# liaoherui/StrainScan

Measured on AMD Instinct MI355X. Metric: M reads/sec vs 1433-strain E. coli DB, higher is better.
Workload: dtype u64

## Files before the change

### strainscan_amd/csrc/ss_reorder.hip

```cpp
#include "ss_common.h"

#include <mutex>
#include "ss_scan_dev.h"

#include <hipcub/hipcub.hpp>

#include <algorithm>
#include <chrono>
#include <vector>

namespace {

constexpr int CH = 64;
constexpr int RB = 256 * CH;
constexpr int HALO = 512;
constexpr int MAX_ORDER_BITS = 22;
constexpr uint32_t NO_NL = 0xFFFFFFFFu;
constexpr int TCAP = 2 * CH;

__device__ __forceinline__ uint32_t nl_mask16(const uint4 v)
{
    const uint32_t w[4] = {v.x, v.y, v.z, v.w};
    uint32_t z[4];
#pragma unroll
// ... 205 lines not shown
        first = false;
        if (!more) break;
        __syncthreads();
    }
}


__device__ __forceinline__ void pad_piece(uint32_t (&w)[4], uint32_t rlen, uint32_t c)
{
    const int keep = (int)min(16u, rlen > c ? rlen - c : 0u);
    if (keep < 16) {
#pragma unroll
        for (int d = 0; d < 4; d++) {
            const int k = keep - 4 * d;
            if (k <= 0) w[d] = 0x0A0A0A0Au;
            else if (k < 4) { const uint32_t m = (1u << (8 * k)) - 1u; w[d] = (w[d] & m) | (0x0A0A0A0Au & ~m); }
        }
    }
}

__device__ __forceinline__ int piece_record(const TileLds &L, uint32_t cnt, uint32_t p)
{
    int lo = 0, hi = (int)cnt - 1;
    while (lo < hi) {
        const int mid = (lo + hi) >> 1;
        if (L.pend[mid] <= p) lo = mid + 1; else hi = mid;
    }
    return lo;
}

__device__ __forceinline__ void store_piece(char *__restrict__ dst, uint64_t out, uint4 v, uint32_t rlen, uint32_t rslot, uint32_t c)
{
    uint32_t w[4] = {v.x, v.y, v.z, v.w};
    pad_piece(w, rlen, c);
    char *o8 = static_cast<char *>(__builtin_assume_aligned(dst + out, 8));
    if (c + 16 <= rslot) __builtin_memcpy(o8, w, 16);
    else __builtin_memcpy(o8, w, 8);
}

__device__ __forceinline__ void copy_round(const char *__restrict__ b, uint64_t n, char *__restrict__ dst, TileLds &L, uint32_t cnt)
{
    const int t = threadIdx.x, lane = t & 63, wave = t >> 6;
    const uint32_t pieces = (uint32_t)t < cnt ? (slot_of(L.len[t]) + 15u) >> 4 : 0u;
    uint32_t pend = wave_incl_sum(pieces, lane);
    if (lane == 63) L.wcnt[wave] = pend;
    __syncthreads();
    uint32_t total = 0;
    for (int w = 0; w < 4; w++) { const uint32_t c = L.wcnt[w]; if (w < wave) pend += c; total += c; }
    if ((uint32_t)t < cnt) L.pend[t] = pend;
    __syncthreads();
    for (uint32_t p = (uint32_t)t; p < total; p += 256) {
        const int lo = piece_record(L, cnt, p);
        const uint32_t rlen = L.len[lo], rslot = slot_of(rlen), c = (p - (L.pend[lo] - ((rslot + 15u) >> 4))) * 16u;
        const uint4 x = rlen > c ? load16_nl(b, L.src[lo] + c, n) : make_uint4(0x0A0A0A0Au, 0x0A0A0A0Au, 0x0A0A0A0Au, 0x0A0A0A0Au);
        store_piece(dst, L.dst[lo] + c, x, rlen, rslot, c);
    }
}

constexpr int PRE = 6;
__global__ __launch_bounds__(256, 8) __attribute__((amdgpu_num_sgpr(80))) void place_kernel(
    const char *__restrict__ b, uint64_t n, unsigned long long *__restrict__ cursor, const uint32_t *__restrict__ tab_cnt,
    const unsigned long long *__restrict__ tab, char *__restrict__ dst)
{
    __shared__ TileLds L;
    const int t = threadIdx.x, lane = t & 63, wave = t >> 6;
    static_assert(TCAP <= 256, "one table entry per thread");
    const unsigned long long e = t < TCAP ? tab[(uint64_t)blockIdx.x * TCAP + t] : 0ull;
    const uint32_t known = tab_cnt[blockIdx.x];
    if (known == T_OVERFLOW || known == 0) return;
    uint64_t d0 = 0;
    uint32_t pieces = 0;
    if ((uint32_t)t < known) {
        const uint32_t len = (uint32_t)(e >> START_BITS) & (LEN_LIMIT - 1u);
        L.src[t] = (uint64_t)blockIdx.x * RB + (uint32_t)(e & (uint32_t)(RB - 1));
        L.len[t] = len;
        d0 = atomicAdd(&cursor[(uint32_t)(e >> (START_BITS + LEN_BITS))], (unsigned long long)slot_of(len));
        pieces = (slot_of(len) + 15u) >> 4;
    }
    uint32_t pend = wave_incl_sum(pieces, lane);
    if (lane == 63) L.wcnt[wave] = pend;
    __syncthreads();
    uint32_t total = 0;
    for (int w = 0; w < 4; w++) { const uint32_t c = L.wcnt[w]; if (w < wave) pend += c; total += c; }
    if ((uint32_t)t < known) L.pend[t] = pend;
    __syncthreads();
    uint4 v[PRE];
    uint32_t rec[PRE], off[PRE];
#pragma unroll
    for (int r = 0; r < PRE; r++) {
        const uint32_t p = (uint32_t)t + 256u * r;
        rec[r] = 0; off[r] = 0;
        v[r] = make_uint4(0x0A0A0A0Au, 0x0A0A0A0Au, 0x0A0A0A0Au, 0x0A0A0A0Au);
        if (p < total) {
            const int lo = piece_record(L, known, p);
            const uint32_t rlen = L.len[lo], c = (p - (L.pend[lo] - ((slot_of(rlen) + 15u) >> 4))) * 16u;
            rec[r] = (uint32_t)lo; off[r] = c;
            if (rlen > c) v[r] = load16_nl(b, L.src[lo] + c, n);
        }
    }
    if ((uint32_t)t < known) L.dst[t] = d0;
    __syncthreads();
#pragma unroll
    for (int r = 0; r < PRE; r++) {
        const uint32_t p = (uint32_t)t + 256u * r;
        if (p < total) {
            const uint32_t rlen = L.len[rec[r]];
            store_piece(dst, L.dst[rec[r]] + off[r], v[r], rlen, slot_of(rlen), off[r]);
        }
    }
    for (uint32_t p = (uint32_t)t + 256u * PRE; p < total; p += 256) {
        const int lo = piece_record(L, known, p);
        const uint32_t rlen = L.len[lo], rslot = slot_of(rlen), c = (p - (L.pend[lo] - ((rslot + 15u) >> 4))) * 16u;
        const uint4 x = rlen > c ? load16_nl(b, L.src[lo] + c, n) : make_uint4(0x0A0A0A0Au, 0x0A0A0A0Au, 0x0A0A0A0Au, 0x0A0A0A0Au);
        store_piece(dst, L.dst[lo] + c, x, rlen, rslot, c);
    }
}

__global__ __launch_bounds__(256) void place_again_kernel(const char *__restrict__ b, uint64_t n, int bits, unsigned long long *__restrict__ cursor,
                                                          const uint32_t *__restrict__ tab_cnt, char *__restrict__ dst)
{
    __shared__ TileLds L;
    const int t = threadIdx.x;
    if (tab_cnt[blockIdx.x] != T_OVERFLOW) return;
    TileState S;
    tile_setup(b, n, L, S);
    while (true) {
        const uint32_t cnt = tile_round(b, n, L, S);
        const bool more = L.more != 0;
        if ((uint32_t)t < cnt) {
            const uint64_t s = L.src[t];
            const uint32_t len = L.len[t];
            const uint32_t bin = (s + 32 <= n) ? record_bin(b, s, len, bits) : (1u << bits);
            L.dst[t] = atomicAdd(&cursor[bin], (unsigned long long)slot_of(len));
        }
        __syncthreads();
        copy_round(b, n, dst, L, cnt);
        if (!more) break;
        __syncthreads();
    }
}

constexpr uint32_t FIX_MIN_L = 32, FIX_MAX_L = 1023;

__device__ __forceinline__ uint32_t not_packable4(uint32_t w)
{
    auto zb = [](uint32_t x) { return ~(((x & 0x7F7F7F7Fu) + 0x7F7F7F7Fu) | x) & 0x80808080u; };
    const uint32_t letter = __builtin_amdgcn_perm(0u, 0x47544341u, (w >> 1) & 0x03030303u);
    return (zb(w ^ letter) | zb(w ^ 0x4E4E4E4Eu) | zb(w ^ 0x0A0A0A0Au)) ^ 0x80808080u;
}

__global__ __launch_bounds__(256, 8) void count_fixed_kernel(const char *__restrict__ b, uint64_t n, uint64_t n_rec, uint32_t L, uint32_t magic_l1, int bits,
                                                             unsigned long long *__restrict__ hist, uint32_t *__restrict__ bins,
                                                             unsigned long long *__restrict__ not_fixed, unsigned long long *__restrict__ not_packable)
{
    const int lane = threadIdx.x & 63;
    const uint64_t r0 = ((uint64_t)blockIdx.x * 4u + (threadIdx.x >> 6)) * 64u;
    if (r0 >= n_rec) return;
    const uint32_t L1 = L + 1u, nr = (uint32_t)min((uint64_t)64, n_rec - r0), span = nr * L1;
    const uint64_t base = r0 * L1;
    bool bad = false;
    uint32_t alpha = 0;
    for (uint32_t off = (uint32_t)lane * 16u; off < span; off += 1024u) {
        const uint4 v = load16_nl(b, base + off, n);
        const uint32_t m = nl_mask16(v);
        const uint32_t pos = off - __umulhi(off, magic_l1) * L1;
        const uint32_t valid = span - off >= 16u ? 0xFFFFu : (1u << (span - off)) - 1u;
        const uint32_t want = L - pos < 16u ? 1u << (L - pos) : 0u;
        bad |= ((m ^ want) & valid) != 0u;
        alpha |= not_packable4(v.x) | not_packable4(v.y) | not_packable4(v.z) | not_packable4(v.w);
    }
    if (r0 + nr == n_rec) {
        for (uint64_t i = base + span + (uint32_t)lane; i < n; i += 64) bad |= b[i] != '\n';
    }
    if (__ballot(bad)) { if (lane == 0) atomicOr(not_fixed, 1ull); return; }
    if (__ballot(alpha != 0u) && lane == 0) atomicOr(not_packable, 1ull);
    if ((uint32_t)lane < nr) {
        const uint32_t bin = record_bin(b, base + (uint64_t)lane * L1, L, bits);
        bins[r0 + lane] = bin;
        atomicAdd(&hist[bin], (unsigned long long)slot_of(L));
    }
}

constexpr int FPRE = 5;
__global__ __launch_bounds__(256, 8) void place_fixed_kernel(const char *__restrict__ b, uint64_t n, uint64_t n_rec, uint32_t L, uint32_t magic_p,
                                                             unsigned long long *__restrict__ cursor, const uint32_t *__restrict__ bins,
                                                             char *__restrict__ dst)
{
    const int lane = threadIdx.x & 63;
    const uint64_t r0 = ((uint64_t)blockIdx.x * 4u + (threadIdx.x >> 6)) * 64u;
    if (r0 >= n_rec) return;
    const uint32_t L1 = L + 1u, nr = (uint32_t)min((uint64_t)64, n_rec - r0), slot = slot_of(L), P = (slot + 15u) >> 4, total = nr * P;
    const uint64_t base = r0 * L1;
    unsigned long long d0 = 0;
    if ((uint32_t)lane < nr) d0 = atomicAdd(&cursor[bins[r0 + lane]], (unsigned long long)slot);
    for (uint32_t p0 = 0; p0 < total; p0 += 64u * FPRE) {
        uint4 v[FPRE];
        uint32_t rec[FPRE], off[FPRE];
#pragma unroll
        for (int r = 0; r < FPRE; r++) {
            const uint32_t p = p0 + (uint32_t)lane + 64u * r;
            rec[r] = min(__umulhi(p, magic_p), nr - 1u);
            off[r] = (p - rec[r] * P) * 16u;
            v[r] = make_uint4(0x0A0A0A0Au, 0x0A0A0A0Au, 0x0A0A0A0Au, 0x0A0A0A0Au);
            if (p < total && L > off[r]) v[r] = load16_nl(b, base + (uint64_t)rec[r] * L1 + off[r], n);
        }
#pragma unroll
        for (int r = 0; r < FPRE; r++) {
            const uint32_t p = p0 + (uint32_t)lane + 64u * r;
            const uint32_t lo = (uint32_t)__shfl((int)(uint32_t)d0, (int)rec[r], 64), hi = (uint32_t)__shfl((int)(uint32_t)(d0 >> 32), (int)rec[r], 64);
            if (p < total) store_piece(dst, (((uint64_t)hi << 32) | lo) + off[r], v[r], L, slot, off[r]);
        }
    }
}

constexpr uint32_t PK_LDS = 4352;
constexpr int FPK = 4;

__global__ __launch_bounds__(256, 6) void place_fixed_packed_kernel(const char *__restrict__ b, uint64_t n, uint64_t n_rec, uint32_t L,
                                                                    uint32_t P, uint32_t magic_p, uint32_t A, uint32_t G, uint32_t ND,
                                                                    uint32_t magic_nd, unsigned long long *__restrict__ cursor,
                                                                    const uint32_t *__restrict__ bins, uint8_t *__restrict__ dst)
{
    __shared__ uint32_t lds[4][PK_LDS / 4 + 1];
    const int lane = threadIdx.x & 63, wave = threadIdx.x >> 6;
    const uint64_t r0 = ((uint64_t)blockIdx.x * 4u + (uint32_t)wave) * 64u;
    if (r0 >= n_rec) return;
    const uint32_t L1 = L + 1u, nr = (uint32_t)min((uint64_t)64, n_rec - r0), slot = slot_of(L), B = slot / 8u * 3u;
    const uint64_t base = r0 * L1;
    uint32_t *W = lds[wave];
    uint8_t *W8 = reinterpret_cast<uint8_t *>(W);
    unsigned long long d0 = 0;
    if ((uint32_t)lane < nr) d0 = atomicAdd(&cursor[bins[r0 + lane]], (unsigned long long)slot);
    for (uint32_t c0 = 0; c0 < nr; c0 += G) {
        const uint32_t nc = min(G, nr - c0), total = nc * P;
        for (uint32_t p0 = 0; p0 < total; p0 += 64u * FPK) {
            uint4 v[FPK];
#pragma unroll
            for (int r = 0; r < FPK; r++) {
                const uint32_t p = p0 + (uint32_t)lane + 64u * r, rec = min(__umulhi(p, magic_p), nc - 1u), off = (p - rec * P) * 16u;
                v[r] = make_uint4(0x0A0A0A0Au, 0x0A0A0A0Au, 0x0A0A0A0Au, 0x0A0A0A0Au);
                if (p < total && L > off) v[r] = load16_nl(b, base + (uint64_t)(c0 + rec) * L1 + off, n);
            }
#pragma unroll
            for (int r = 0; r < FPK; r++) {
                const uint32_t p = p0 + (uint32_t)lane + 64u * r, rec = min(__umulhi(p, magic_p), nc - 1u), off = (p - rec * P) * 16u;
                if (p >= total) continue;
                uint32_t w[4] = {v[r].x, v[r].y, v[r].z, v[r].w};
                pad_piece(w, L, off);
                uint32_t code, inv;
                ss::dev::encode16(w, code, inv);
                uint16_t *q = reinterpret_cast<uint16_t *>(W8 + rec * A + 4u + (off >> 4) * 6u);
                q[0] = (uint16_t)code;
                q[1] = (uint16_t)((inv & 0xFFu) | ((code >> 8) & 0xFF00u));
                q[2] = (uint16_t)((code >> 24) | (inv & 0xFF00u));
            }
        }
        __builtin_amdgcn_fence(__ATOMIC_RELEASE, "wavefront");
        __builtin_amdgcn_wave_barrier();
        __builtin_amdgcn_fence(__ATOMIC_ACQUIRE, "wavefront");
        const uint32_t items = nc * ND;
        for (uint32_t i0 = 0; i0 < items; i0 += 64u) {
            const uint32_t i = i0 + (uint32_t)lane, rec = min(__umulhi(i, magic_nd), nc - 1u), jl = i - rec * ND;
            const uint32_t lo = (uint32_t)__shfl((int)(uint32_t)d0, (int)(c0 + rec), 64), hi = (uint32_t)__shfl((int)(uint32_t)(d0 >> 32), (int)(c0 + rec), 64);
            const uint64_t D = ((((uint64_t)hi << 32) | lo) >> 3) * 3u;
            const int o = (int)(4u * jl) - (int)(D & 3u);
            if (i < items && o < (int)B) {
                const uint32_t x = rec * A + 4u + (uint32_t)o;
                const uint32_t val = __builtin_amdgcn_alignbyte(W[(x >> 2) + 1u], W[x >> 2], x & 3u);
                uint8_t *out = dst + (D & ~3ull) + 4u * jl;
                if (o >= 0 && o + 4 <= (int)B) {
                    *reinterpret_cast<uint32_t *>(__builtin_assume_aligned(out, 4)) = val;
                } else {
#pragma unroll
                    for (int k = 0; k < 4; k++)
                        if (o + k >= 0 && o + k < (int)B) out[k] = (uint8_t)(val >> (8 * k));
                }
            }
        }
        __builtin_amdgcn_fence(__ATOMIC_RELEASE, "wavefront");
        __builtin_amdgcn_wave_barrier();
        __builtin_amdgcn_fence(__ATOMIC_ACQUIRE, "wavefront");
    }
}

__global__ __launch_bounds__(256) void key_fixed_kernel(const char *__restrict__ b, uint64_t n, uint64_t n_rec, uint32_t L, int bits,
                                                        uint32_t *__restrict__ key, uint32_t *__restrict__ val,
                                                        unsigned long long *__restrict__ not_fixed)
{
    const uint64_t i = (uint64_t)blockIdx.x * 256u + threadIdx.x;
    if (i >= n_rec) return;
    const uint64_t s = i * (L + 1u);
    bool bad = i > 0 && b[s - 1] != '\n';
    if (i + 1 == n_rec)
        for (uint64_t k = s + L; k < n; k++) bad |= b[k] != '\n';
    key[i] = record_bin(b, s, L, bits);
    val[i] = (uint32_t)i;
    const uint64_t m = __ballot(bad);
    if (m && (uint32_t)(threadIdx.x & 63) == (uint32_t)__builtin_ctzll(m) &&
        !*(volatile unsigned long long *)not_fixed) atomicOr(not_fixed, 1ull);
}

constexpr uint32_t GX_LDS_PK = 6144, GX_LDS_ASCII = 8192;
constexpr int GPK = 3;

inline uint32_t gather_rows(bool pk, uint32_t L)
{
    const uint32_t slot = slot_of(L), R = pk ? slot / 8u * 3u : slot, lim = pk ? GX_LDS_PK : GX_LDS_ASCII;
    uint32_t G = 64;
    while (G > 1 && (G * R > lim || (G * R) % 16u)) G--;
    return G;
}

template <bool PK>
__global__ __launch_bounds__(256, 7) void gather_fixed_kernel(const char *__restrict__ b, uint64_t n, uint64_t n_rec, uint32_t L,
                                                              uint32_t P, uint32_t magic_p, uint32_t G, const uint32_t *__restrict__ perm,
                                                              uint8_t *__restrict__ dst, unsigned long long *__restrict__ not_fixed,
                                                              unsigned long long *__restrict__ not_packable)
{
    extern __shared__ uint4 gx_lds[];
    const int lane = threadIdx.x & 63, wave = threadIdx.x >> 6;
    const uint64_t r0 = ((uint64_t)blockIdx.x * 4u + (uint32_t)wave) * 64u;
    if (r0 >= n_rec || *(volatile unsigned long long *)not_fixed || (PK && *(volatile unsigned long long *)not_packable)) return;
    const uint32_t L1 = L + 1u, nr = (uint32_t)min((uint64_t)64, n_rec - r0), slot = slot_of(L), R = PK ? slot / 8u * 3u : slot;
    uint4 *W = gx_lds + (size_t)wave * (G * R / 16u);
    uint8_t *W8 = reinterpret_cast<uint8_t *>(W);
    const uint32_t mine = (uint32_t)lane < nr ? perm[r0 + lane] : 0u;
    bool bad = false;
    uint32_t alpha = 0;
    for (uint32_t c0 = 0; c0 < nr; c0 += G) {
        const uint32_t nc = min(G, nr - c0), total = nc * P;
        for (uint32_t p0 = 0; p0 < total; p0 += 64u * GPK) {
            uint4 v[GPK];
#pragma unroll
            for (int r = 0; r < GPK; r++) {
                const uint32_t p = p0 + (uint32_t)lane + 64u * r, rec = min(__umulhi(p, magic_p), nc - 1u), off = (p - rec * P) * 16u;
                const uint32_t s = (uint32_t)__shfl((int)mine, (int)(c0 + rec), 64);
                v[r] = make_uint4(0x0A0A0A0Au, 0x0A0A0A0Au, 0x0A0A0A0Au, 0x0A0A0A0Au);
                if (p < total && L >= off) v[r] = load16_clamped(b, (uint64_t)s * L1 + off, n);
            }
#pragma unroll
            for (int r = 0; r < GPK; r++) {
                const uint32_t p = p0 + (uint32_t)lane + 64u * r, rec = min(__umulhi(p, magic_p), nc - 1u), off = (p - rec * P) * 16u;
                if (p >= total) continue;
                uint32_t w[4] = {v[r].x, v[r].y, v[r].z, v[r].w};
                if (L >= off) {
                    const uint32_t m = nl_mask16(v[r]), e = L - off;
                    const uint32_t want = e < 16u ? 1u << e : 0u, valid = e < 16u ? (2u << e) - 1u : 0xFFFFu;
                    bad |= ((m ^ want) & valid) != 0u;
                }
                const int keep = (int)min(16u, L > off ? L - off : 0u);
                if (keep < 16) {
#pragma unroll
                    for (int d = 0; d < 4; d++) {
                        const int k = keep - 4 * d;
                        if (k <= 0) w[d] = 0x0A0A0A0Au;
                        else if (k < 4) { const uint32_t mk = (1u << (8 * k)) - 1u; w[d] = (w[d] & mk) | (0x0A0A0A0Au & ~mk); }
                    }
                }
                if (PK) {
                    alpha |= not_packable4(w[0]) | not_packable4(w[1]) | not_packable4(w[2]) | not_packable4(w[3]);
                    uint32_t code, inv;
                    ss::dev::encode16(w, code, inv);
                    uint8_t *q = W8 + rec * R + (off >> 4) * 6u;
                    q[0] = (uint8_t)code; q[1] = (uint8_t)(code >> 8); q[2] = (uint8_t)inv;
                    if (off + 16u <= slot) { q[3] = (uint8_t)(code >> 16); q[4] = (uint8_t)(code >> 24); q[5] = (uint8_t)(inv >> 8); }
                } else {
                    uint64_t *q = reinterpret_cast<uint64_t *>(W8 + rec * R + off);
                    q[0] = (uint64_t)w[0] | ((uint64_t)w[1] << 32);
                    if (off + 16u <= slot) q[1] = (uint64_t)w[2] | ((uint64_t)w[3] << 32);
                }
            }
        }
        __builtin_amdgcn_fence(__ATOMIC_RELEASE, "wavefront");
        __builtin_amdgcn_wave_barrier();
        __builtin_amdgcn_fence(__ATOMIC_ACQUIRE, "wavefront");
        const uint32_t span = nc * R;
        uint8_t *out = dst + (r0 + c0) * R;
        for (uint32_t q = (uint32_t)lane * 16u; q < span; q += 1024u) {
            if (q + 16u <= span) *reinterpret_cast<uint4 *>(__builtin_assume_aligned(out + q, 16)) = W[q >> 4];
            else for (uint32_t k = q; k < span; k++) out[k] = W8[k];
        }
        __builtin_amdgcn_fence(__ATOMIC_RELEASE, "wavefront");
        __builtin_amdgcn_wave_barrier();
        __builtin_amdgcn_fence(__ATOMIC_ACQUIRE, "wavefront");
    }
    if (__ballot(bad) && lane == 0 && !*(volatile unsigned long long *)not_fixed) atomicOr(not_fixed, 1ull);
    if (PK && __ballot(alpha != 0u) && lane == 0 && !*(volatile unsigned long long *)not_packable) atomicOr(not_packable, 1ull);
}

constexpr int SCAN_PER = 4096;

__global__ __launch_bounds__(1024) void scan_sums_kernel(const unsigned long long *__restrict__ v, uint32_t n, unsigned long long *__restrict__ sums)
{
    __shared__ unsigned long long s_w[16];
    const int t = threadIdx.x, lane = t & 63, wave = t >> 6;
    const uint32_t i0 = blockIdx.x * SCAN_PER + (uint32_t)t * 4u;
    unsigned long long x = 0;
    for (uint32_t i = i0; i < min(n, i0 + 4u); i++) x += v[i];
#pragma unroll
    for (int off = 32; off > 0; off >>= 1) x += (unsigned long long)__shfl_xor((long long)x, off, 64);
    if (lane == 0) s_w[wave] = x;
    __syncthreads();
    if (t == 0) { unsigned long long r = 0; for (int w = 0; w < 16; w++) r += s_w[w]; sums[blockIdx.x] = r; }
}

__global__ __launch_bounds__(1024) void scan_top_kernel(unsigned long long *__restrict__ sums, uint32_t nb, unsigned long long *__restrict__ total)
{
    __shared__ unsigned long long s_part[1024];
    const int t = threadIdx.x;
    const uint32_t per = (nb + 1023u) / 1024u, a = min(nb, (uint32_t)t * per), e = min(nb, a + per);
    unsigned long long sum = 0;
    for (uint32_t i = a; i < e; i++) sum += sums[i];
    s_part[t] = sum;
    __syncthreads();
    if (t == 0) {
        unsigned long long run = 0;
        for (int i = 0; i < 1024; i++) { const unsigned long long v = s_part[i]; s_part[i] = run; run += v; }
        *total = run;
    }
    __syncthreads();
    unsigned long long run = s_part[t];
    for (uint32_t i = a; i < e; i++) { const unsigned long long v = sums[i]; sums[i] = run; run += v; }
}

__global__ __launch_bounds__(1024) void scan_apply_kernel(unsigned long long *__restrict__ v, uint32_t n, const unsigned long long *__restrict__ sums)
{
    __shared__ unsigned long long s_w[16];
    const int t = threadIdx.x, lane = t & 63, wave = t >> 6;
    const uint32_t i0 = blockIdx.x * SCAN_PER + (uint32_t)t * 4u;
    unsigned long long x[4], mine = 0;
#pragma unroll
    for (int k = 0; k < 4; k++) { x[k] = i0 + k < n ? v[i0 + k] : 0ull; mine += x[k]; }
    unsigned long long incl = mine;
#pragma unroll
    for (int off = 1; off < 64; off <<= 1) {
        const unsigned long long o = (unsigned long long)__shfl_up((long long)incl, off, 64);
        if (lane >= off) incl += o;
    }
    if (lane == 63) s_w[wave] = incl;
    __syncthreads();
    unsigned long long run = sums[blockIdx.x] + incl - mine;
    for (int w = 0; w < wave; w++) run += s_w[w];
#pragma unroll
    for (int k = 0; k < 4; k++) { if (i0 + k < n) v[i0 + k] = run; run += x[k]; }
}

int order_bits(uint64_t n_bytes)
{
    int bits = 12;
    while (bits < MAX_ORDER_BITS && (n_bytes / 152) >> (bits + 2)) bits++;
    return bits;
}

}

namespace ss {

static std::mutex g_scr_mu;
static uint64_t g_order_n[2] = {0, 0};
static double g_order_ms[3] = {0, 0, 0};
static char *g_scr = nullptr;
static uint64_t g_scr_cap = 0;

std::atomic<long long> g_hook_ascii_slabs{0};
std::atomic<long long> g_hook_atomic_binning{0};

namespace {

typedef std::chrono::steady_clock Clock;
inline double ms_between(Clock::time_point a, Clock::time_point b) { return std::chrono::duration<double, std::milli>(b - a).count(); }

enum class Binned { done, not_one_length, failed };
enum { T_TOTAL = 0, T_FLAG = 1, T_ALPHA = 2 };

inline bool hip_ok(hipError_t e, const char *what, int line)
{
    if (e != hipSuccess) ss::set_last_error(what, __FILE__, line, hipGetLastError());
    return e == hipSuccess;
}
#define SS_R(call) do { if (!hip_ok((call), #call, __LINE__)) return Binned::failed; } while (0)
struct Owner { Owner() = default; Owner(const Owner &) = delete; Owner &operator=(const Owner &) = delete; };

struct Call {
    const char *src;
    uint64_t n;
    int bits;
    uint32_t n_bins;
    unsigned nb, nsb;
    Clock::time_point t_begin = Clock::now();
    Call(const char *src_, uint64_t n_) : src(src_), n(n_), bits(order_bits(n_)), n_bins((1u << bits) + 1u), nb((unsigned)((n_ + RB - 1) / RB)),
                                          nsb((n_bins + SCAN_PER - 1) / SCAN_PER) {}
    void lap(const char *what) const
    {
        static const bool trace = getenv("SS_INGEST_TRACE") != nullptr;
        if (!trace) return;
        hipDeviceSynchronize();
        fprintf(stderr, "[reorder] %-22s at %.4f s\n", what, std::chrono::duration<double>(Clock::now() - t_begin).count());
    }
    hipError_t finish(Clock::time_point *t_end) const
    {
        hipError_t e = hipGetLastError();
        if (e == hipSuccess) e = hipDeviceSynchronize();
        lap("place");
        *t_end = Clock::now();
        return e;
    }
};

struct OneLength { uint32_t L = 0; uint64_t n_rec = 0; };

hipError_t probe_one_length(const char *src, uint64_t n, OneLength *one)
{
    *one = OneLength();
    static const bool fixed_allowed = [] { const char *e = getenv("SS_ORDER_FIXED"); return !(e && !strcmp(e, "0")); }();
    if (!fixed_allowed || n < 64) return hipSuccess;
    char head[FIX_MAX_L + 2];
    const size_t hn = (size_t)std::min<uint64_t>(n, sizeof(head));
    const hipError_t e = hipMemcpy(head, src, hn, hipMemcpyDeviceToHost);
    if (e != hipSuccess) return e;
    const void *nl = memchr(head, '\n', hn);
    if (!nl) return hipSuccess;
    const uint32_t L = (uint32_t)((const char *)nl - head);
    if (L >= FIX_MIN_L && L <= FIX_MAX_L && n / (L + 1) >= 1 && n - (n / (L + 1)) * (L + 1) < 64) { one->L = L; one->n_rec = n / (L + 1); }
    return hipSuccess;
}

class Scratch : Owner {
public:
    struct Sort { uint32_t *k0, *k1, *v0, *v1; void *temp; size_t temp_bytes; };
    ~Scratch() { if (d_) hipFree(d_); }

    hipError_t take(const Call &c, const OneLength &one, bool for_sort)
    {
        n_bins_ = c.n_bins;
        if (for_sort) {
            hipcub::DoubleBuffer<uint32_t> k(nullptr, nullptr), v(nullptr, nullptr);
            const hipError_t e = hipcub::DeviceRadixSort::SortPairs(nullptr, sort_tb_, k, v, (int)one.n_rec, 0, c.bits + 1);
            if (e != hipSuccess) return e;
        }
        a4_ = (one.n_rec * 4 + 255) & ~255ull;
        o_sums_ = ((uint64_t)c.n_bins + 3) * 8;
        o_cnt_ = o_sums_ + ((uint64_t)c.nsb + 1) * 8;
        o_region_ = (o_cnt_ + (uint64_t)c.nb * 4 + 255) & ~255ull;
        const uint64_t bytes = o_region_ + std::max<uint64_t>((uint64_t)c.nb * TCAP * 8, for_sort ? 4 * a4_ + ((sort_tb_ + 255) & ~255ull) : a4_);
        {
            std::lock_guard<std::mutex> g(g_scr_mu);
            if (g_scr && g_scr_cap >= bytes) { d_ = g_scr; cap_ = g_scr_cap; g_scr = nullptr; g_scr_cap = 0; }
        }
        if (d_) return hipSuccess;
        cap_ = bytes;
        return hipMalloc((void **)&d_, bytes);
    }
    void keep()
    {
        {
            std::lock_guard<std::mutex> g(g_scr_mu);
            if (!g_scr || g_scr_cap < cap_) { std::swap(g_scr, d_); std::swap(g_scr_cap, cap_); }
        }
        if (d_) hipFree(d_);
        d_ = nullptr;
    }

    unsigned long long *hist() const { return (unsigned long long *)d_; }
    unsigned long long *tail() const { return hist() + n_bins_; }
    uint64_t hist_bytes() const { return o_sums_; }
    unsigned long long *sums() const { return (unsigned long long *)(d_ + o_sums_); }
    uint32_t *tile_counts() const { return (uint32_t *)(d_ + o_cnt_); }
    unsigned long long *table() const { return (unsigned long long *)(d_ + o_region_); }
    uint32_t *bins() const { return (uint32_t *)(d_ + o_region_); }
    Sort sort() const
    {
        uint32_t *a = (uint32_t *)(d_ + o_region_);
        return Sort{a, a + a4_ / 4, a + 2 * (a4_ / 4), a + 3 * (a4_ / 4), d_ + o_region_ + 4 * a4_, sort_tb_};
    }

private:
    char *d_ = nullptr;
    uint64_t cap_ = 0, o_sums_ = 0, o_cnt_ = 0, o_region_ = 0, a4_ = 0;
    uint32_t n_bins_ = 0;
    size_t sort_tb_ = 0;
};

struct NewSlab : Owner {
    char *d = nullptr;
    uint64_t total = 0, cap = 0, real_cap = 0;
    bool packed = false;
    Clock::time_point t_alloc;
    ~NewSlab() { if (d) hipFree(d); }

    hipError_t alloc(const Call &c, bool pk, uint64_t total_)
    {
        total = total_; packed = pk;
        cap = std::max<uint64_t>((total + 15) & ~15ull, 16);
        const hipError_t e = get_block();
        t_alloc = Clock::now();
        c.lap("new slab");
        return e;
    }
    hipError_t make_ascii()
    {
        packed = false;
        if (real_cap >= cap) return hipSuccess;
        put_back();
        return get_block();
    }
    hipError_t fill_tail() const
    {
        hipError_t e = hipSuccess;
        if (packed) {
            const uint64_t t0 = total / 8u * 3u, t1 = ss::dev::in_bytes(true, cap) + 8;
            e = hipMemsetAsync(d + t0, 0xFF, t1 - t0, 0);
            if (e == hipSuccess && cap > total) e = hipMemsetAsync(d + t0, 0x55, 2, 0);
        } else if (cap > total) {
            e = hipMemsetAsync(d + total, '\n', cap - total, 0);
        }
        return e;
    }
    void put_back() { ss::big_put(d, real_cap); d = nullptr; }
    char *release() { char *p = d; d = nullptr; return p; }

private:
    hipError_t get_block()
    {
        const uint64_t bytes = packed ? std::max<uint64_t>(ss::dev::in_bytes(true, cap) + 8, cap >= ss::BIG_KEEP_MIN ? cap : 0) : cap;
        return ss::big_malloc((void **)&d, bytes, &real_cap);
    }
};

struct EventPair : Owner {
    hipEvent_t ev[2] = {nullptr, nullptr};
    ~EventPair() { for (hipEvent_t e : ev) if (e) hipEventDestroy(e); }
    hipError_t create() { const hipError_t e = hipEventCreate(&ev[0]); return e == hipSuccess ? hipEventCreate(&ev[1]) : e; }
};

hipError_t prefix_and_tail(const Call &c, const Scratch &scr, unsigned long long *tail, int n_tail)
{
    hipLaunchKernelGGL(scan_sums_kernel, dim3(c.nsb), dim3(1024), 0, 0, scr.hist(), c.n_bins, scr.sums());
    hipLaunchKernelGGL(scan_top_kernel, dim3(1), dim3(1024), 0, 0, scr.sums(), c.nsb, scr.tail());
    hipLaunchKernelGGL(scan_apply_kernel, dim3(c.nsb), dim3(1024), 0, 0, scr.hist(), c.n_bins, scr.sums());
    return hipMemcpy(tail, scr.tail(), 8 * (size_t)n_tail, hipMemcpyDeviceToHost);
}

hipError_t finish_counted(const Call &c, Clock::time_point t_counted, const NewSlab &slab, double ms[3])
{
    Clock::time_point t_end;
    const hipError_t e = c.finish(&t_end);
    ms[0] = ms_between(c.t_begin, t_counted); ms[1] = ms_between(t_counted, slab.t_alloc); ms[2] = ms_between(slab.t_alloc, t_end);
    return e;
}

Binned bin_sorted(const Call &c, const OneLength &one, const Scratch &scr, NewSlab &slab, double ms[3])
{
    const uint32_t slot = ::slot_of(one.L), P = (slot + 15u) >> 4;
    const unsigned nbf = (unsigned)((one.n_rec + 255) / 256);
    SS_R(slab.alloc(c, g_hook_ascii_slabs.load() == 0, one.n_rec * slot));
    const Scratch::Sort s = scr.sort();
    unsigned long long *flags = scr.tail();
    EventPair t;
    SS_R(t.create());
    auto gather = [&](const uint32_t *perm) {
        const uint32_t G = gather_rows(slab.packed, one.L), R = slab.packed ? slot / 8u * 3u : slot;
        auto kern = slab.packed ? gather_fixed_kernel<true> : gather_fixed_kernel<false>;
        hipLaunchKernelGGL(kern, dim3(nbf), dim3(256), 4u * G * R, 0, c.src, c.n, one.n_rec, one.L, P, (uint32_t)(((1ull << 32) + P - 1) / P), G,
                           perm, (uint8_t *)slab.d, flags + T_FLAG, flags + T_ALPHA);
    };
    unsigned long long tail[3] = {0, 0, 0};
    SS_R(hipMemsetAsync(flags, 0, 24, 0));
    SS_R(hipEventRecord(t.ev[0], 0));
    hipLaunchKernelGGL(key_fixed_kernel, dim3(nbf), dim3(256), 0, 0, c.src, c.n, one.n_rec, one.L, c.bits, s.k0, s.v0, flags + T_FLAG);
    hipcub::DoubleBuffer<uint32_t> dk(s.k0, s.k1), dv(s.v0, s.v1);
    size_t temp_bytes = s.temp_bytes;
    SS_R(hipcub::DeviceRadixSort::SortPairs(s.temp, temp_bytes, dk, dv, (int)one.n_rec, 0, c.bits + 1, 0));
    SS_R(hipEventRecord(t.ev[1], 0));
    const uint32_t *perm = dv.Current();
    gather(perm);
    SS_R(slab.fill_tail());
    SS_R(hipMemcpy(tail + T_FLAG, flags + T_FLAG, 16, hipMemcpyDeviceToHost));
    if (tail[T_FLAG] == 0 && slab.packed && tail[T_ALPHA]) {
        SS_R(slab.make_ascii());
        gather(perm);
        SS_R(slab.fill_tail());
        SS_R(hipMemcpy(tail + T_FLAG, flags + T_FLAG, 8, hipMemcpyDeviceToHost));
    }
    SS_R(hipGetLastError());
    if (tail[T_FLAG]) { slab.put_back(); return Binned::not_one_length; }
    float ms_key_sort = -1.f;
    SS_R(hipEventElapsedTime(&ms_key_sort, t.ev[0], t.ev[1]));
    Clock::time_point t_end;
    SS_R(c.finish(&t_end));
    ms[0] = ms_key_sort; ms[1] = ms_between(c.t_begin, slab.t_alloc); ms[2] = ms_between(slab.t_alloc, t_end) - ms_key_sort;
    return Binned::done;
}

Binned bin_counted(const Call &c, const OneLength &one, const Scratch &scr, NewSlab &slab, double ms[3])
{
    const uint32_t L1 = one.L + 1u, slot = ::slot_of(one.L), P = (slot + 15u) >> 4;
    const unsigned nbf = (unsigned)((one.n_rec + 255) / 256);
    unsigned long long tail[3] = {0, 0, 0};
    SS_R(hipMemsetAsync(scr.hist(), 0, scr.hist_bytes(), 0));
    hipLaunchKernelGGL(count_fixed_kernel, dim3(nbf), dim3(256), 0, 0, c.src, c.n, one.n_rec, one.L, (uint32_t)(((1ull << 32) + L1 - 1) / L1), c.bits,
                       scr.hist(), scr.bins(), scr.tail() + T_FLAG, scr.tail() + T_ALPHA);
    SS_R(prefix_and_tail(c, scr, tail, 3));
    if (tail[T_FLAG]) return Binned::not_one_length;
    c.lap("count + prefix");
    const Clock::time_point t_counted = Clock::now();
    SS_R(slab.alloc(c, tail[T_ALPHA] == 0 && g_hook_ascii_slabs.load() == 0, tail[T_TOTAL]));
    if (slab.packed) {
        const uint32_t B = slot / 8u * 3u, A = (6u * P + 8u + 3u) & ~3u;
        const uint32_t G = std::min<uint32_t>(64u, PK_LDS / A), ND = ((B + 2u) >> 2) + 1u;
        hipLaunchKernelGGL(place_fixed_packed_kernel, dim3(nbf), dim3(256), 0, 0, c.src, c.n, one.n_rec, one.L, P, (uint32_t)(((1ull << 32) + P - 1) / P),
                           A, G, ND, (uint32_t)(((1ull << 32) + ND - 1) / ND), scr.hist(), (const uint32_t *)scr.bins(), (uint8_t *)slab.d);
    } else {
        hipLaunchKernelGGL(place_fixed_kernel, dim3(nbf), dim3(256), 0, 0, c.src, c.n, one.n_rec, one.L, (uint32_t)(((1ull << 32) + P - 1) / P),
                           scr.hist(), (const uint32_t *)scr.bins(), slab.d);
    }
    SS_R(slab.fill_tail());
    SS_R(finish_counted(c, t_counted, slab, ms));
    return Binned::done;
}

Binned bin_general(const Call &c, const Scratch &scr, NewSlab &slab, double ms[3])
{
    unsigned long long tail[2] = {0, 0};
    SS_R(hipMemsetAsync(scr.hist(), 0, scr.hist_bytes(), 0));
    hipLaunchKernelGGL(count_kernel, dim3(c.nb), dim3(256), 0, 0, c.src, c.n, c.bits, scr.hist(), scr.tile_counts(), scr.table(), scr.tail() + T_FLAG);
    SS_R(prefix_and_tail(c, scr, tail, 2));
    c.lap("count + prefix");
    const Clock::time_point t_counted = Clock::now();
    SS_R(slab.alloc(c, false, tail[T_TOTAL]));
    hipLaunchKernelGGL(place_kernel, dim3(c.nb), dim3(256), 0, 0, c.src, c.n, scr.hist(), scr.tile_counts(), scr.table(), slab.d);
    if (tail[T_FLAG]) hipLaunchKernelGGL(place_again_kernel, dim3(c.nb), dim3(256), 0, 0, c.src, c.n, c.bits, scr.hist(), scr.tile_counts(), slab.d);
    SS_R(slab.fill_tail());
    SS_R(finish_counted(c, t_counted, slab, ms));
    return Binned::done;
}
#undef SS_R

}

int order_flat_dev(const char *src, uint64_t n, ss_reads::Slab *out)
{
    *out = ss_reads::Slab();
    const Call c(src, n);
    OneLength one;
    if (!hip_ok(probe_one_length(src, n, &one), "hipMemcpy", __LINE__)) return SS_EHIP;
    const bool sorted = one.L && g_hook_atomic_binning.load() == 0 && one.n_rec < (1ull << 31);
    Scratch scr;
    if (!hip_ok(scr.take(c, one, sorted), "Scratch::take", __LINE__)) return SS_EHIP;
    NewSlab slab;
    double ms[3] = {0, 0, 0};
    Binned r = Binned::not_one_length;
    if (one.L) r = sorted ? bin_sorted(c, one, scr, slab, ms) : bin_counted(c, one, scr, slab, ms);
    const bool fixed = r == Binned::done;
    if (r == Binned::not_one_length) r = bin_general(c, scr, slab, ms);
    if (r != Binned::done) return SS_EHIP;
    {
        std::lock_guard<std::mutex> g(g_scr_mu);
        for (int i = 0; i < 3; i++) g_order_ms[i] = ms[i];
        g_order_n[fixed ? 0 : 1]++;
    }
    scr.keep();
    out->cap = slab.real_cap; out->binned = true;
    out->used = slab.packed ? ss::dev::in_bytes(true, slab.cap) : slab.cap;
    if (slab.packed) { out->packed = true; out->n_pos = slab.cap; out->L = one.L; out->slot = ::slot_of(one.L); }
    out->d = slab.release();
    return SS_OK;
}

void reorder_timing(double out[3])
{
    std::lock_guard<std::mutex> g(g_scr_mu);
    for (int i = 0; i < 3; i++) out[i] = g_order_ms[i];
}

void reorder_counters(uint64_t out[2])
{
    std::lock_guard<std::mutex> g(g_scr_mu);
    out[0] = g_order_n[0]; out[1] = g_order_n[1];
}

void reorder_release()
{
    char *d = nullptr;
    {
        std::lock_guard<std::mutex> g(g_scr_mu);
        std::swap(d, g_scr);
        g_scr_cap = 0;
    }
    if (d) hipFree(d);
}

bool reads_order_wanted()
{
    const char *e = getenv("SS_READS_ORDER");
    return !(e && (!strcmp(e, "file") || !strcmp(e, "0") || !strcmp(e, "off")));
}

int reads_order_for_locality(ss_reads *R, bool force)
{
    if (!R) return SS_EINVAL;
    if (!force && !reads_order_wanted()) return SS_OK;
    uint64_t bytes = 0;
    size_t mem_free = 0, mem_total = 0;
    const bool known = hipMemGetInfo(&mem_free, &mem_total) == hipSuccess;
    for (auto &sl : R->slabs) {
        const bool room = known && mem_free > sl.used + sl.used / 8 + (1ull << 30);
        if (sl.used >= 64 && (room || force)) {
            ss_reads::Slab nsl;
            const int rc = order_flat_dev(sl.d, sl.used, &nsl);
            if (rc) return rc;
            ss::big_put(sl.d, sl.cap);
            sl = nsl;
        }
        bytes += sl.cap;
    }
    R->device_bytes = bytes;
    return SS_OK;
}

}
```

Before: 3078.

## Pack reads before sorting, then gather compact packed rows by permutation

```diff
diff --git a/strainscan_amd/csrc/ss_reorder.hip b/strainscan_amd/csrc/ss_reorder.hip
--- a/strainscan_amd/csrc/ss_reorder.hip
+++ b/strainscan_amd/csrc/ss_reorder.hip
@@ -531,31 +531,177 @@
 
 constexpr uint32_t GX_LDS_PK = 6144, GX_LDS_ASCII = 8192;
 constexpr int GPK = 3;
+constexpr int PKP = 2;
+constexpr int GQ = 4;
+
+__host__ __device__ __forceinline__ uint32_t packed_row(uint32_t slot) { return slot / 8u * 3u; }
+__host__ __device__ __forceinline__ uint32_t packed_stride(uint32_t slot) { return (packed_row(slot) + 15u) & ~15u; }
 
 inline uint32_t gather_rows(bool pk, uint32_t L)
 {
-    const uint32_t slot = slot_of(L), R = pk ? slot / 8u * 3u : slot, lim = pk ? GX_LDS_PK : GX_LDS_ASCII;
+    const uint32_t slot = slot_of(L), R = pk ? packed_row(slot) : slot, lim = pk ? GX_LDS_PK : GX_LDS_ASCII;
     uint32_t G = 64;
     while (G > 1 && (G * R > lim || (G * R) % 16u)) G--;
     return G;
 }
-
-template <bool PK>
-__global__ __launch_bounds__(256, 7) void gather_fixed_kernel(const char *__restrict__ b, uint64_t n, uint64_t n_rec, uint32_t L,
-                                                              uint32_t P, uint32_t magic_p, uint32_t G, const uint32_t *__restrict__ perm,
-                                                              uint8_t *__restrict__ dst, unsigned long long *__restrict__ not_fixed,
-                                                              unsigned long long *__restrict__ not_packable)
+inline uint32_t pack_rows(uint32_t L) { return std::min<uint32_t>(64u, GX_LDS_PK / packed_stride(slot_of(L))); }
+
+typedef uint32_t u32x4 __attribute__((ext_vector_type(4)));
+__device__ __forceinline__ uint4 load16_once(const void *p)
+{
+    const u32x4 x = __builtin_nontemporal_load(static_cast<const u32x4 *>(__builtin_assume_aligned(p, 16)));
+    return make_uint4(x.x, x.y, x.z, x.w);
+}
+__device__ __forceinline__ void store16_once(void *p, const uint4 v)
+{
+    const u32x4 x = {v.x, v.y, v.z, v.w};
+    __builtin_nontemporal_store(x, static_cast<u32x4 *>(__builtin_assume_aligned(p, 16)));
+}
+
+__global__ __launch_bounds__(256, 8) void pack_key_fixed_kernel(const char *__restrict__ b, uint64_t n, uint64_t n_rec, uint32_t L, uint32_t P,
+                                                                uint32_t magic_p, uint32_t G, int bits, uint32_t *__restrict__ key,
+                                                                uint32_t *__restrict__ val, uint8_t *__restrict__ inter,
+                                                                unsigned long long *__restrict__ not_fixed, unsigned long long *__restrict__ not_packable)
 {
     extern __shared__ uint4 gx_lds[];
     const int lane = threadIdx.x & 63, wave = threadIdx.x >> 6;
     const uint64_t r0 = ((uint64_t)blockIdx.x * 4u + (uint32_t)wave) * 64u;
-    if (r0 >= n_rec || *(volatile unsigned long long *)not_fixed || (PK && *(volatile unsigned long long *)not_packable)) return;
-    const uint32_t L1 = L + 1u, nr = (uint32_t)min((uint64_t)64, n_rec - r0), slot = slot_of(L), R = PK ? slot / 8u * 3u : slot;
+    if (r0 >= n_rec || __ballot(*(volatile unsigned long long *)not_fixed != 0ull)) return;
+    const bool pack = __ballot(*(volatile unsigned long long *)not_packable != 0ull) == 0ull;
+    const uint32_t L1 = L + 1u, nr = (uint32_t)min((uint64_t)64, n_rec - r0), slot = slot_of(L), Rt = packed_stride(slot);
+    const uint64_t base = r0 * L1;
+    uint4 *W = gx_lds + (size_t)wave * (G * Rt / 16u);
+    uint8_t *W8 = reinterpret_cast<uint8_t *>(W);
+    bool bad = false;
+    uint32_t alpha = 0;
+    for (uint32_t c0 = 0; pack && c0 < nr; c0 += G) {
+        const uint32_t nc = min(G, nr - c0), total = nc * P;
+        for (uint32_t p0 = 0; p0 < total; p0 += 64u * PKP) {
+            uint4 v[PKP];
+#pragma unroll
+            for (int r = 0; r < PKP; r++) {
+                const uint32_t p = p0 + (uint32_t)lane + 64u * r, rec = min(__umulhi(p, magic_p), nc - 1u), off = (p - rec * P) * 16u;
+                v[r] = make_uint4(0x0A0A0A0Au, 0x0A0A0A0Au, 0x0A0A0A0Au, 0x0A0A0A0Au);
+                if (p < total && L >= off) v[r] = load16_clamped(b, base + (uint64_t)(c0 + rec) * L1 + off, n);
+            }
+#pragma unroll
+            for (int r = 0; r < PKP; r++) {
+                const uint32_t p = p0 + (uint32_t)lane + 64u * r, rec = min(__umulhi(p, magic_p), nc - 1u), off = (p - rec * P) * 16u;
+                if (p >= total) continue;
+                uint32_t w[4] = {v[r].x, v[r].y, v[r].z, v[r].w};
+                if (L >= off) {
+                    const uint32_t m = nl_mask16(v[r]), e = L - off;
+                    const uint32_t want = e < 16u ? 1u << e : 0u, valid = e < 16u ? (2u << e) - 1u : 0xFFFFu;
+                    bad |= ((m ^ want) & valid) != 0u;
+                }
+                pad_piece(w, L, off);
+                alpha |= not_packable4(w[0]) | not_packable4(w[1]) | not_packable4(w[2]) | not_packable4(w[3]);
+                uint32_t code, inv;
+                ss::dev::encode16(w, code, inv);
+                uint16_t *q = reinterpret_cast<uint16_t *>(W8 + rec * Rt + (off >> 4) * 6u);
+                q[0] = (uint16_t)code;
+                q[1] = (uint16_t)((inv & 0xFFu) | ((code >> 8) & 0xFF00u));
+                if (off + 16u <= slot) q[2] = (uint16_t)((code >> 24) | (inv & 0xFF00u));
+            }
+        }
+        __builtin_amdgcn_fence(__ATOMIC_RELEASE, "wavefront");
+        __builtin_amdgcn_wave_barrier();
+        __builtin_amdgcn_fence(__ATOMIC_ACQUIRE, "wavefront");
+        uint8_t *out = inter + (r0 + c0) * Rt;
+        for (uint32_t q = (uint32_t)lane * 16u; q < nc * Rt; q += 1024u) store16_once(out + q, W[q >> 4]);
+        __builtin_amdgcn_fence(__ATOMIC_RELEASE, "wavefront");
+        __builtin_amdgcn_wave_barrier();
+        __builtin_amdgcn_fence(__ATOMIC_ACQUIRE, "wavefront");
+    }
+    if (r0 + nr == n_rec) {
+        for (uint64_t i = base + (uint64_t)nr * L1 + (uint32_t)lane; i < n; i += 64) bad |= b[i] != '\n';
+    }
+    if (__ballot(bad)) { if (lane == 0 && !*(volatile unsigned long long *)not_fixed) atomicOr(not_fixed, 1ull); return; }
+    if (__ballot(alpha != 0u) && lane == 0 && !*(volatile unsigned long long *)not_packable) atomicOr(not_packable, 1ull);
+    if ((uint32_t)lane < nr) {
+        key[r0 + lane] = record_bin(b, base + (uint64_t)lane * L1, L, bits);
+        val[r0 + lane] = (uint32_t)(r0 + lane);
+    }
+}
+
+__global__ __launch_bounds__(256, 8) void gather_packed_kernel(const uint8_t *__restrict__ inter, uint64_t n_rec, uint32_t R, uint32_t magic_r,
+                                                               uint32_t Q, uint32_t magic_q, uint32_t G, const uint32_t *__restrict__ perm,
+                                                               uint8_t *__restrict__ dst, const unsigned long long *__restrict__ not_fixed,
+                                                               const unsigned long long *__restrict__ not_packable)
+{
+    extern __shared__ uint4 gx_lds[];
+    const int lane = threadIdx.x & 63, wave = threadIdx.x >> 6;
+    const uint64_t r0 = ((uint64_t)blockIdx.x * 4u + (uint32_t)wave) * 64u;
+    if (r0 >= n_rec || *(volatile const unsigned long long *)not_fixed || *(volatile const unsigned long long *)not_packable) return;
+    const uint32_t nr = (uint32_t)min((uint64_t)64, n_rec - r0), Rt = Q * 16u;
+    uint4 *W = gx_lds + (size_t)wave * (G * Q + 1u);
+    const uint32_t *W32 = reinterpret_cast<const uint32_t *>(W);
+    const uint8_t *W8 = reinterpret_cast<const uint8_t *>(W);
+    const uint32_t mine = (uint32_t)lane < nr ? min(perm[r0 + lane], (uint32_t)(n_rec - 1u)) : 0u;
+    for (uint32_t c0 = 0; c0 < nr; c0 += G) {
+        const uint32_t nc = min(G, nr - c0), total = nc * Q;
+        for (uint32_t p0 = 0; p0 < total; p0 += 64u * GQ) {
+            uint4 v[GQ];
+#pragma unroll
+            for (int r = 0; r < GQ; r++) {
+                const uint32_t p = p0 + (uint32_t)lane + 64u * r, rec = min(Q == 1u ? p : __umulhi(p, magic_q), nc - 1u), k = p - rec * Q;
+                const uint32_t s = (uint32_t)__shfl((int)mine, (int)(c0 + rec), 64);
+                v[r] = make_uint4(0u, 0u, 0u, 0u);
+                if (p < total) v[r] = load16_once(inter + (uint64_t)s * Rt + k * 16u);
+            }
+#pragma unroll
+            for (int r = 0; r < GQ; r++) {
+                const uint32_t p = p0 + (uint32_t)lane + 64u * r;
+                if (p < total) W[p] = v[r];
+            }
+        }
+        __builtin_amdgcn_fence(__ATOMIC_RELEASE, "wavefront");
+        __builtin_amdgcn_wave_barrier();
+        __builtin_amdgcn_fence(__ATOMIC_ACQUIRE, "wavefront");
+        const uint32_t span = nc * R;
+        uint8_t *out = dst + (r0 + c0) * R;
+        for (uint32_t q = (uint32_t)lane * 16u; q < span; q += 1024u) {
+            uint32_t rec = __umulhi(q, magic_r), o = q - rec * R;
+            if (q + 16u <= span) {
+                uint32_t w[4];
+#pragma unroll
+                for (int d = 0; d < 4; d++) {
+                    const uint32_t x = rec * Rt + o;
+                    w[d] = __builtin_amdgcn_alignbyte(W32[(x >> 2) + 1u], W32[x >> 2], x & 3u);
+                    if (o + 4u > R) {
+                        const uint32_t keep = 8u * (R - o);
+                        w[d] = (w[d] & ((1u << keep) - 1u)) | (W32[((rec + 1u) * Rt) >> 2] << keep);
+                    }
+                    o += 4u;
+                    if (o >= R) { o -= R; rec++; }
+                }
+                store16_once(out + q, make_uint4(w[0], w[1], w[2], w[3]));
+            } else {
+                for (uint32_t k = q; k < span; k++) {
+                    out[k] = W8[rec * Rt + o];
+                    if (++o == R) { o = 0; rec++; }
+                }
+            }
+        }
+        __builtin_amdgcn_fence(__ATOMIC_RELEASE, "wavefront");
+        __builtin_amdgcn_wave_barrier();
+        __builtin_amdgcn_fence(__ATOMIC_ACQUIRE, "wavefront");
+    }
+}
+
+__global__ __launch_bounds__(256, 8) void gather_fixed_kernel(const char *__restrict__ b, uint64_t n, uint64_t n_rec, uint32_t L,
+                                                              uint32_t P, uint32_t magic_p, uint32_t G, const uint32_t *__restrict__ perm,
+                                                              uint8_t *__restrict__ dst, unsigned long long *__restrict__ not_fixed)
+{
+    extern __shared__ uint4 gx_lds[];
+    const int lane = threadIdx.x & 63, wave = threadIdx.x >> 6;
+    const uint64_t r0 = ((uint64_t)blockIdx.x * 4u + (uint32_t)wave) * 64u;
+    if (r0 >= n_rec || *(volatile unsigned long long *)not_fixed) return;
+    const uint32_t L1 = L + 1u, nr = (uint32_t)min((uint64_t)64, n_rec - r0), slot = slot_of(L), R = slot;
     uint4 *W = gx_lds + (size_t)wave * (G * R / 16u);
     uint8_t *W8 = reinterpret_cast<uint8_t *>(W);
     const uint32_t mine = (uint32_t)lane < nr ? perm[r0 + lane] : 0u;
     bool bad = false;
-    uint32_t alpha = 0;
     for (uint32_t c0 = 0; c0 < nr; c0 += G) {
         const uint32_t nc = min(G, nr - c0), total = nc * P;
         for (uint32_t p0 = 0; p0 < total; p0 += 64u * GPK) {
@@ -577,27 +723,10 @@
                     const uint32_t want = e < 16u ? 1u << e : 0u, valid = e < 16u ? (2u << e) - 1u : 0xFFFFu;
                     bad |= ((m ^ want) & valid) != 0u;
                 }
-                const int keep = (int)min(16u, L > off ? L - off : 0u);
-                if (keep < 16) {
-#pragma unroll
-                    for (int d = 0; d < 4; d++) {
-                        const int k = keep - 4 * d;
-                        if (k <= 0) w[d] = 0x0A0A0A0Au;
-                        else if (k < 4) { const uint32_t mk = (1u << (8 * k)) - 1u; w[d] = (w[d] & mk) | (0x0A0A0A0Au & ~mk); }
-                    }
-                }
-                if (PK) {
-                    alpha |= not_packable4(w[0]) | not_packable4(w[1]) | not_packable4(w[2]) | not_packable4(w[3]);
-                    uint32_t code, inv;
-                    ss::dev::encode16(w, code, inv);
-                    uint8_t *q = W8 + rec * R + (off >> 4) * 6u;
-                    q[0] = (uint8_t)code; q[1] = (uint8_t)(code >> 8); q[2] = (uint8_t)inv;
-                    if (off + 16u <= slot) { q[3] = (uint8_t)(code >> 16); q[4] = (uint8_t)(code >> 24); q[5] = (uint8_t)(inv >> 8); }
-                } else {
-                    uint64_t *q = reinterpret_cast<uint64_t *>(W8 + rec * R + off);
-                    q[0] = (uint64_t)w[0] | ((uint64_t)w[1] << 32);
-                    if (off + 16u <= slot) q[1] = (uint64_t)w[2] | ((uint64_t)w[3] << 32);
-                }
+                pad_piece(w, L, off);
+                uint64_t *q = reinterpret_cast<uint64_t *>(W8 + rec * R + off);
+                q[0] = (uint64_t)w[0] | ((uint64_t)w[1] << 32);
+                if (off + 16u <= slot) q[1] = (uint64_t)w[2] | ((uint64_t)w[3] << 32);
             }
         }
         __builtin_amdgcn_fence(__ATOMIC_RELEASE, "wavefront");
@@ -614,7 +743,6 @@
         __builtin_amdgcn_fence(__ATOMIC_ACQUIRE, "wavefront");
     }
     if (__ballot(bad) && lane == 0 && !*(volatile unsigned long long *)not_fixed) atomicOr(not_fixed, 1ull);
-    if (PK && __ballot(alpha != 0u) && lane == 0 && !*(volatile unsigned long long *)not_packable) atomicOr(not_packable, 1ull);
 }
 
 constexpr int SCAN_PER = 4096;
@@ -754,12 +882,29 @@
     return hipSuccess;
 }
 
+inline uint64_t slab_positions(uint64_t total) { return std::max<uint64_t>((total + 15) & ~15ull, 16); }
+inline uint64_t packed_block_bytes(uint64_t cap) { return std::max<uint64_t>(ss::dev::in_bytes(true, cap) + 8, cap >= ss::BIG_KEEP_MIN ? cap : 0); }
+struct PackPlan {
+    uint64_t bytes = 0, slab_off = 0;
+    bool in_slab = false, large = false;
+    uint64_t scratch_bytes() const { return in_slab ? 0 : bytes; }
+    explicit PackPlan(const OneLength &one)
+    {
+        if (!one.L) return;
+        const uint64_t cap = slab_positions(one.n_rec * ::slot_of(one.L));
+        bytes = one.n_rec * packed_stride(::slot_of(one.L));
+        slab_off = (ss::dev::in_bytes(true, cap) + 8 + 255) & ~255ull;
+        in_slab = slab_off + bytes <= packed_block_bytes(cap);
+        large = cap >= ss::BIG_KEEP_MIN;
+    }
+};
+
 class Scratch : Owner {
 public:
     struct Sort { uint32_t *k0, *k1, *v0, *v1; void *temp; size_t temp_bytes; };
     ~Scratch() { if (d_) hipFree(d_); }
 
-    hipError_t take(const Call &c, const OneLength &one, bool for_sort)
+    hipError_t take(const Call &c, const OneLength &one, bool for_sort, uint64_t inter_bytes, bool inter_of_large_slab)
     {
         n_bins_ = c.n_bins;
         if (for_sort) {
@@ -771,7 +916,9 @@
         o_sums_ = ((uint64_t)c.n_bins + 3) * 8;
         o_cnt_ = o_sums_ + ((uint64_t)c.nsb + 1) * 8;
         o_region_ = (o_cnt_ + (uint64_t)c.nb * 4 + 255) & ~255ull;
-        const uint64_t bytes = o_region_ + std::max<uint64_t>((uint64_t)c.nb * TCAP * 8, for_sort ? 4 * a4_ + ((sort_tb_ + 255) & ~255ull) : a4_);
+        o_inter_ = o_region_ + 4 * a4_ + ((sort_tb_ + 255) & ~255ull);
+        const uint64_t bytes = std::max<uint64_t>(o_region_ + std::max<uint64_t>((uint64_t)c.nb * TCAP * 8, a4_), for_sort ? o_inter_ + inter_bytes : 0);
+        transient_ = for_sort && inter_bytes && inter_of_large_slab;
         {
             std::lock_guard<std::mutex> g(g_scr_mu);
             if (g_scr && g_scr_cap >= bytes) { d_ = g_scr; cap_ = g_scr_cap; g_scr = nullptr; g_scr_cap = 0; }
@@ -782,7 +929,7 @@
     }
     void keep()
     {
-        {
+        if (!transient_) {
             std::lock_guard<std::mutex> g(g_scr_mu);
             if (!g_scr || g_scr_cap < cap_) { std::swap(g_scr, d_); std::swap(g_scr_cap, cap_); }
         }
@@ -802,12 +949,14 @@
         uint32_t *a = (uint32_t *)(d_ + o_region_);
         return Sort{a, a + a4_ / 4, a + 2 * (a4_ / 4), a + 3 * (a4_ / 4), d_ + o_region_ + 4 * a4_, sort_tb_};
     }
+    uint8_t *intermediate() const { return (uint8_t *)(d_ + o_inter_); }
 
 private:
     char *d_ = nullptr;
-    uint64_t cap_ = 0, o_sums_ = 0, o_cnt_ = 0, o_region_ = 0, a4_ = 0;
+    uint64_t cap_ = 0, o_sums_ = 0, o_cnt_ = 0, o_region_ = 0, o_inter_ = 0, a4_ = 0;
     uint32_t n_bins_ = 0;
     size_t sort_tb_ = 0;
+    bool transient_ = false;
 };
 
 struct NewSlab : Owner {
@@ -820,7 +969,7 @@
     hipError_t alloc(const Call &c, bool pk, uint64_t total_)
     {
         total = total_; packed = pk;
-        cap = std::max<uint64_t>((total + 15) & ~15ull, 16);
+        cap = slab_positions(total);
         const hipError_t e = get_block();
         t_alloc = Clock::now();
         c.lap("new slab");
@@ -851,7 +1000,7 @@
 private:
     hipError_t get_block()
     {
-        const uint64_t bytes = packed ? std::max<uint64_t>(ss::dev::in_bytes(true, cap) + 8, cap >= ss::BIG_KEEP_MIN ? cap : 0) : cap;
+        const uint64_t bytes = packed ? packed_block_bytes(cap) : cap;
         return ss::big_malloc((void **)&d, bytes, &real_cap);
     }
 };
@@ -878,36 +1027,49 @@
     return e;
 }
 
-Binned bin_sorted(const Call &c, const OneLength &one, const Scratch &scr, NewSlab &slab, double ms[3])
-{
-    const uint32_t slot = ::slot_of(one.L), P = (slot + 15u) >> 4;
+Binned bin_sorted(const Call &c, const OneLength &one, bool want_packed, const PackPlan &plan, const Scratch &scr, NewSlab &slab, double ms[3])
+{
+    const uint32_t slot = ::slot_of(one.L), P = (slot + 15u) >> 4, magic_p = (uint32_t)(((1ull << 32) + P - 1) / P);
     const unsigned nbf = (unsigned)((one.n_rec + 255) / 256);
-    SS_R(slab.alloc(c, g_hook_ascii_slabs.load() == 0, one.n_rec * slot));
+    SS_R(slab.alloc(c, want_packed, one.n_rec * slot));
     const Scratch::Sort s = scr.sort();
     unsigned long long *flags = scr.tail();
     EventPair t;
     SS_R(t.create());
-    auto gather = [&](const uint32_t *perm) {
-        const uint32_t G = gather_rows(slab.packed, one.L), R = slab.packed ? slot / 8u * 3u : slot;
-        auto kern = slab.packed ? gather_fixed_kernel<true> : gather_fixed_kernel<false>;
-        hipLaunchKernelGGL(kern, dim3(nbf), dim3(256), 4u * G * R, 0, c.src, c.n, one.n_rec, one.L, P, (uint32_t)(((1ull << 32) + P - 1) / P), G,
-                           perm, (uint8_t *)slab.d, flags + T_FLAG, flags + T_ALPHA);
+    auto gather_ascii = [&](const uint32_t *perm) {
+        const uint32_t G = gather_rows(false, one.L);
+        hipLaunchKernelGGL(gather_fixed_kernel, dim3(nbf), dim3(256), 4u * G * slot, 0, c.src, c.n, one.n_rec, one.L, P, magic_p, G, perm,
+                           (uint8_t *)slab.d, flags + T_FLAG);
     };
+    const bool packing = slab.packed;
+    uint8_t *inter = !packing ? nullptr : plan.in_slab ? (uint8_t *)slab.d + plan.slab_off : scr.intermediate();
     unsigned long long tail[3] = {0, 0, 0};
     SS_R(hipMemsetAsync(flags, 0, 24, 0));
     SS_R(hipEventRecord(t.ev[0], 0));
-    hipLaunchKernelGGL(key_fixed_kernel, dim3(nbf), dim3(256), 0, 0, c.src, c.n, one.n_rec, one.L, c.bits, s.k0, s.v0, flags + T_FLAG);
+    if (packing) {
+        const uint32_t G = pack_rows(one.L);
+        hipLaunchKernelGGL(pack_key_fixed_kernel, dim3(nbf), dim3(256), 4u * G * packed_stride(slot), 0, c.src, c.n, one.n_rec, one.L, P, magic_p, G,
+                           c.bits, s.k0, s.v0, inter, flags + T_FLAG, flags + T_ALPHA);
+    } else {
+        hipLaunchKernelGGL(key_fixed_kernel, dim3(nbf), dim3(256), 0, 0, c.src, c.n, one.n_rec, one.L, c.bits, s.k0, s.v0, flags + T_FLAG);
+    }
     hipcub::DoubleBuffer<uint32_t> dk(s.k0, s.k1), dv(s.v0, s.v1);
     size_t temp_bytes = s.temp_bytes;
     SS_R(hipcub::DeviceRadixSort::SortPairs(s.temp, temp_bytes, dk, dv, (int)one.n_rec, 0, c.bits + 1, 0));
     SS_R(hipEventRecord(t.ev[1], 0));
     const uint32_t *perm = dv.Current();
-    gather(perm);
+    if (packing) {
+        const uint32_t G = gather_rows(true, one.L), R = packed_row(slot), Q = packed_stride(slot) / 16u;
+        hipLaunchKernelGGL(gather_packed_kernel, dim3(nbf), dim3(256), 4u * (G * Q + 1u) * 16u, 0, inter, one.n_rec, R, (uint32_t)(((1ull << 32) + R - 1) / R),
+                           Q, (uint32_t)(((1ull << 32) + Q - 1) / Q), G, perm, (uint8_t *)slab.d, flags + T_FLAG, flags + T_ALPHA);
+    } else {
+        gather_ascii(perm);
+    }
     SS_R(slab.fill_tail());
     SS_R(hipMemcpy(tail + T_FLAG, flags + T_FLAG, 16, hipMemcpyDeviceToHost));
-    if (tail[T_FLAG] == 0 && slab.packed && tail[T_ALPHA]) {
+    if (tail[T_FLAG] == 0 && packing && tail[T_ALPHA]) {
         SS_R(slab.make_ascii());
-        gather(perm);
+        gather_ascii(perm);
         SS_R(slab.fill_tail());
         SS_R(hipMemcpy(tail + T_FLAG, flags + T_FLAG, 8, hipMemcpyDeviceToHost));
     }
@@ -974,12 +1136,14 @@
     OneLength one;
     if (!hip_ok(probe_one_length(src, n, &one), "hipMemcpy", __LINE__)) return SS_EHIP;
     const bool sorted = one.L && g_hook_atomic_binning.load() == 0 && one.n_rec < (1ull << 31);
+    const bool want_packed = g_hook_ascii_slabs.load() == 0;
+    const PackPlan plan(one);
     Scratch scr;
-    if (!hip_ok(scr.take(c, one, sorted), "Scratch::take", __LINE__)) return SS_EHIP;
+    if (!hip_ok(scr.take(c, one, sorted, sorted && want_packed ? plan.scratch_bytes() : 0, plan.large), "Scratch::take", __LINE__)) return SS_EHIP;
     NewSlab slab;
     double ms[3] = {0, 0, 0};
     Binned r = Binned::not_one_length;
-    if (one.L) r = sorted ? bin_sorted(c, one, scr, slab, ms) : bin_counted(c, one, scr, slab, ms);
+    if (one.L) r = sorted ? bin_sorted(c, one, want_packed, plan, scr, slab, ms) : bin_counted(c, one, scr, slab, ms);
     const bool fixed = r == Binned::done;
     if (r == Binned::not_one_length) r = bin_general(c, scr, slab, ms);
     if (r != Binned::done) return SS_EHIP;
```

Result: faster. 3239, median of 6 (+5.2%).
